# zxhuang1698/ZeroShape

Hardware: AMD Instinct MI355X
Metric: sdf_query_points_per_sec_vox128 (higher is better)
Workload: dtype f16x3

## Files before the change

include/zeroshape_hip.h:

```cpp
#ifndef ZEROSHAPE_HIP_H
#define ZEROSHAPE_HIP_H

#include <stddef.h>
#include <stdint.h>

#ifdef __cplusplus
extern "C" {
#endif

#define ZS_ABI_VERSION 40

int zs_abi_version(void);

const char *zs_last_error(void);


int zs_chamfer_forward(const float *xyz1, const float *xyz2, int b, int n, int m,
                       float *dist1, float *dist2, int *idx1, int *idx2, void *stream);

size_t zs_chamfer_workspace_bytes(int b, int n, int m);
int zs_chamfer_forward_ws(const float *xyz1, const float *xyz2, int b, int n, int m,
                          float *dist1, float *dist2, int *idx1, int *idx2,
                          void *workspace, size_t workspace_bytes, void *stream);

int zs_chamfer_backward(const float *xyz1, const float *xyz2, int b, int n, int m,
// ... 32 lines not shown
                           const float *axis, int G, const int *columns, int n_cols, float *zmean,
                           void *workspace, void *scratch, size_t scratch_bytes, void *stream);

int zs_attn_frames(const float *zmean, int batch, int n_cols, const int *frame_col, int n_frames,
                   const float *images, int H, int W, const uint8_t *lut, int R, float *frames, void *stream);

int zs_sdf_split_programs(const void *programs, size_t program_stride_bytes, void *split_programs,
                          size_t split_stride_bytes, int batch, void *stream);
int zs_sdf_query_points_split(const void *split_programs, size_t program_stride_bytes, int batch,
                              const float *points, int m, float *logits, int *tile_flags,
                              void *workspace, void *stream);
int zs_sdf_query_grid_split(const void *split_programs, size_t program_stride_bytes, int batch,
                            const float *axis, int G, int slice_begin, int slice_end,
                            int apply_sigmoid, float *out, int *tile_flags, void *workspace,
                            void *stream);

int zs_sdf_query_grid_range(const void *programs, size_t program_stride_bytes, int batch,
                            const float *axis, int G, long long point_begin, long long point_end,
                            int apply_sigmoid, float *out, const int *tile_mask, void *workspace,
                            void *stream);
int zs_sdf_query_grid_range_split(const void *split_programs, size_t program_stride_bytes, int batch,
                                  const float *axis, int G, long long point_begin,
                                  long long point_end, int apply_sigmoid, float *out,
                                  int *tile_flags, void *workspace, void *stream);

size_t zs_bf_grid_bytes(void);
size_t zs_bf_scratch_bytes(void);
int zs_bf_lower_bounds(const float *pred, int n, const float *gt_normalized, int m,
                       const float *rotations, int k, float *grid_gt, float *grid_pred,
                       void *scratch, float *lower_bounds, void *stream);
// ... 283 lines not shown
```

zeroshape_amd/_lib.py:

```python
import contextlib
import ctypes
import os

_HERE = os.path.dirname(os.path.abspath(__file__))
LIB_PATH = os.environ.get("ZS_LIB_PATH") or os.path.join(_HERE, "libzeroshape_hip.so")

_c_void_p = ctypes.c_void_p
_c_int = ctypes.c_int
_c_size_t = ctypes.c_size_t
_c_float = ctypes.c_float

class ConvFuse(ctypes.Structure):
    _fields_ = [("in_mode", ctypes.c_int), ("in_tiles", ctypes.c_int), ("in_groups", ctypes.c_int), ("in_gshift", ctypes.c_int),
                ("in_stats", ctypes.c_void_p), ("in_gamma", ctypes.c_void_p), ("in_beta", ctypes.c_void_p),
                ("in_eps", ctypes.c_float), ("out_mode", ctypes.c_int), ("out_groups", ctypes.c_int),
                ("out_stats", ctypes.c_void_p)]


SIGNATURES = {
    "zs_abi_version": (_c_int, []),
    "zs_last_error": (ctypes.c_char_p, []),
    "zs_chamfer_forward": (_c_int, [_c_void_p, _c_void_p, _c_int, _c_int, _c_int,
                                    _c_void_p, _c_void_p, _c_void_p, _c_void_p, _c_void_p]),
    "zs_chamfer_workspace_bytes": (_c_size_t, [_c_int, _c_int, _c_int]),
# ... 13 lines not shown
                                    _c_void_p, _c_int, _c_void_p]),
    "zs_sdf_verdict_stats": (_c_int, [_c_void_p, _c_void_p, _c_int, _c_int, _c_float, _c_float, _c_float, _c_void_p, _c_void_p,
                                      _c_void_p]),
    "zs_sdf_query_points": (_c_int, [_c_void_p, _c_size_t, _c_int, _c_void_p, _c_int,
                                     _c_void_p, _c_void_p, _c_void_p, _c_void_p, _c_void_p]),
    "zs_sdf_query_grid": (_c_int, [_c_void_p, _c_size_t, _c_int, _c_void_p, _c_int, _c_int,
                                   _c_int, _c_int, _c_void_p, _c_void_p, _c_void_p, _c_void_p]),
    "zs_sdf_grid_attn_zmean_scratch_bytes": (_c_size_t, [_c_int, _c_int, _c_int, _c_size_t]),
    "zs_sdf_grid_attn_zmean_chunk": (_c_int, [_c_int, _c_int, _c_int, _c_size_t, ctypes.POINTER(_c_int),
                                              ctypes.POINTER(_c_int)]),
    "zs_sdf_grid_attn_zmean": (_c_int, [_c_void_p, _c_size_t, _c_int, _c_void_p, _c_int, _c_void_p, _c_int, _c_void_p,
                                        _c_void_p, _c_void_p, _c_size_t, _c_void_p]),
    "zs_attn_frames": (_c_int, [_c_void_p, _c_int, _c_int, _c_void_p, _c_int, _c_void_p, _c_int, _c_int, _c_void_p, _c_int,
                                _c_void_p, _c_void_p]),
    "zs_sdf_split_programs": (_c_int, [_c_void_p, _c_size_t, _c_void_p, _c_size_t, _c_int, _c_void_p]),
    "zs_sdf_query_points_split": (_c_int, [_c_void_p, _c_size_t, _c_int, _c_void_p, _c_int,
                                           _c_void_p, _c_void_p, _c_void_p, _c_void_p]),
    "zs_sdf_query_grid_split": (_c_int, [_c_void_p, _c_size_t, _c_int, _c_void_p, _c_int, _c_int,
                                         _c_int, _c_int, _c_void_p, _c_void_p, _c_void_p, _c_void_p]),
    "zs_sdf_query_grid_range": (_c_int, [_c_void_p, _c_size_t, _c_int, _c_void_p, _c_int, ctypes.c_longlong,
                                         ctypes.c_longlong, _c_int, _c_void_p, _c_void_p, _c_void_p, _c_void_p]),
    "zs_sdf_query_grid_range_split": (_c_int, [_c_void_p, _c_size_t, _c_int, _c_void_p, _c_int,
                                               ctypes.c_longlong, ctypes.c_longlong, _c_int, _c_void_p,
                                               _c_void_p, _c_void_p, _c_void_p]),
    "zs_erode_mask": (_c_int, [_c_void_p, _c_int, _c_int, _c_int, _c_int, _c_void_p, _c_void_p]),
    "zs_bf_grid_bytes": (_c_size_t, []),
    "zs_bf_scratch_bytes": (_c_size_t, []),
    "zs_bf_lower_bounds": (_c_int, [_c_void_p, _c_int, _c_void_p, _c_int, _c_void_p, _c_int, _c_void_p,
                                    _c_void_p, _c_void_p, _c_void_p, _c_void_p]),
    "zs_pose_max_batch": (_c_int, []),
# ... 129 lines not shown
    "zs_group_norm_bwd_workspace_bytes": (_c_size_t, [_c_int, _c_int]),
    "zs_group_norm_bwd": (_c_int, [_c_void_p] * 8 + [_c_int, _c_int, _c_int, _c_int, _c_float, _c_void_p, _c_void_p]),
    "zs_max_pool_bwd_nhwc": (_c_int, [_c_void_p] * 3 + [_c_int] * 10 + [_c_void_p]),
    "zs_global_mean_bwd_nhwc": (_c_int, [_c_void_p, _c_void_p, _c_int, _c_int, _c_int, _c_void_p]),
    "zs_upsample2x_bwd_nhwc": (_c_int, [_c_void_p, _c_void_p, _c_int, _c_int, _c_int, _c_int, _c_void_p]),
    "zs_nhwc_to_nchw_masked": (_c_int, [_c_void_p, _c_void_p, _c_void_p, _c_int, _c_int, _c_int, _c_int, _c_void_p]),
    "zs_seen_surface_bwd": (_c_int, [_c_void_p] * 7 + [_c_int, _c_int, _c_int, _c_void_p, _c_void_p, _c_void_p]),
    "zs_intr_param2mtx_bwd": (_c_int, [_c_void_p, _c_void_p, _c_int, _c_int, _c_int, _c_void_p, _c_void_p]),
    "zs_window_tokens_bwd": (_c_int, [_c_void_p] * 5 + [_c_int] * 5 + [_c_void_p]),
    "zs_coord_dsp2_bwd": (_c_int, [_c_void_p] * 4 + [_c_int] * 3 + [_c_void_p]),
    "zs_transform_points": (_c_int, [_c_void_p] * 5 + [_c_int, _c_int, _c_void_p]),
    "zs_resize_bilinear_nhwc": (_c_int, [_c_void_p, _c_void_p] + [_c_int] * 6 + [_c_void_p]),
    "zs_readout_concat_bwd": (_c_int, [_c_void_p, _c_void_p, _c_int, _c_int, _c_int, _c_void_p]),
}

ABI_VERSION = 40
_lib = None


class ZeroShapeHipError(RuntimeError):
    pass


def load():
    global _lib
    if _lib is not None:
        return _lib
    if not os.path.exists(LIB_PATH):
        raise ZeroShapeHipError(
            "HIP library not built: %s is missing (run `python -m zeroshape_amd.build`). "
            "zeroshape_amd has no CPU/PyTorch fallback for this path." % LIB_PATH)
# ... 51 lines not shown
```

zeroshape_amd/csrc/sdf_decoder_split.hip:

```cpp
#include "zs_common.h"
#include <stdlib.h>
#include "sdf_layout.h"
#include "sdf_math.h"
#include "zs_split16.h"
#include "../../include/zeroshape_hip.h"

#include <math.h>
#include <stdint.h>
#include <type_traits>

namespace {

using namespace zs::lay;
using zs::dm::gelu_erf;
using zs::dm::softplus100;

typedef float f32x16 __attribute__((ext_vector_type(16)));
typedef float f32x4 __attribute__((ext_vector_type(4)));
typedef float f32x2 __attribute__((ext_vector_type(2)));
typedef unsigned u32x4 __attribute__((ext_vector_type(4)));

constexpr float S_GUARD = 64.0f;
constexpr int WAVES = 4;
constexpr int PTS_PER_WAVE = 32;
// ... 63 lines not shown
    asm volatile("s_mov_b32 m0, %1\n\ts_nop 0\n\tglobal_load_lds_dwordx4 %0, off" ZS_DMA_MOD
                 "\n\tglobal_load_lds_dwordx4 %0, off offset:1024" ZS_DMA_MOD
                 "\n\tglobal_load_lds_dwordx4 %0, off offset:2048" ZS_DMA_MOD
                 "\n\tglobal_load_lds_dwordx4 %0, off offset:3072" ZS_DMA_MOD
                 :
                 : "v"(gsrc), "s"(lds_dst)
                 : "memory");
}

struct AStream {
    const u32x4 *buf[NBUF];
    unsigned dst[NBUF];
    u32x4 hi, lo;
    const char *gsrc;

    DEV void init(const char *prog, u32x4 *stage, unsigned stage_addr, int wave, int lane) {
        const char *g = prog + wave * (KPW * KB_U4 * 16) + lane * 16;
        asm volatile("s_waitcnt vmcnt(0) lgkmcnt(0)\n\ts_barrier" ::: "memory");
#pragma unroll
        for (int i = 0; i < NBUF; i++) {
            buf[i] = stage + i * (CK * KB_U4) + lane;
            dst[i] = stage_addr + i * CHUNK_BYTES + wave * (KPW * KB_U4 * 16);
            glds_kblocks(g + i * CHUNK_BYTES, dst[i]);
        }
        gsrc = g + NBUF * CHUNK_BYTES;
        asm volatile("s_waitcnt vmcnt(4)\n\ts_barrier" ::: "memory");
        hi = buf[0][0];
        lo = buf[0][64];
    }
    template <int EXTRA_VM = 0>
    DEV void step(int pos, u32x4 &ahi, u32x4 &alo) {
        ahi = hi;
// ... 9 lines not shown
            const u32x4 *t = buf[0];
            const unsigned u = dst[0];
            buf[0] = buf[1];
            dst[0] = dst[1];
            buf[1] = t;
            dst[1] = u;
            hi = buf[0][0];
            lo = buf[0][64];
        } else {
#ifndef ZS_EXP_NO_AREAD
            hi = buf[0][(pos + 1) * KB_U4];
            lo = buf[0][(pos + 1) * KB_U4 + 64];
#endif
        }
    }
    DEV void drain() { asm volatile("s_waitcnt vmcnt(0) lgkmcnt(0)" ::: "memory"); }
};

struct Slab {
    u32x4 *fl;
    PT t7;
    DEV void store(int tile, const PT &p) {
        if (tile == SLAB_TILES) {
            t7 = p;
        } else {
#pragma unroll
            for (int q = 0; q < 4; q++) fl[(tile * 4 + q) * 64] = p.v[q];
        }
    }
};
// ... 124 lines not shown
#endif
                 "v_mul_f32_e64 %[t], |%[x]|, %[c0]\n\t"
                 "v_exp_f32_e32 %[t], %[t]\n\t"
                 "v_mfma_f32_32x32x16_f16 %[acc], %[ahi], %[bl], %[acc]\n\t"
                 "v_max_f32_e32 %[m], 0, %[x]\n\t"
                 "v_add_f32_e32 %[t], 1.0, %[t]\n\t"
                 "v_log_f32_e32 %[t], %[t]\n\t"
                 "v_mfma_f32_32x32x16_f16 %[acc], %[ahi], %[bh], %[acc]\n\t"
                 "s_nop 0\n\t"
                 "v_fmac_f32_e32 %[m], 0x3be32166, %[t]"
                 : [acc] "+v"(acc), [t] "=&v"(t), [m] "=&v"(m)
                 : [alo] "v"(alo), [ahi] "v"(ahi), [bh] "v"(bhi), [bl] "v"(blo), [x] "v"(x), [c0] "s"(c0));
    return m;
}

template <int KT, int EXTRA_VM = 0, typename SIDE = NoSide>
DEV void gemm_reg(AStream &s, const PT *X, f32x16 &acc, SIDE side = SIDE()) {
#pragma unroll
    for (int kt = 0; kt < KT; kt++)
#pragma unroll
        for (int j = 0; j < 2; j++) {
            u32x4 ahi, alo;
            s.step((kt * 2 + j) & (CK - 1), ahi, alo);
            pin(ahi, alo);
            mfma3_gaps(acc, ahi, alo, X[kt].v[2 * j], X[kt].v[2 * j + 1], kt * 2 + j, side);
        }
}
template <typename SIDE>
DEV void mfma3_breg(f32x16 &acc, const u32x4 &ahi, const u32x4 &alo, const u32x4 &bhi, const u32x4 &blo, int kb,
                    SIDE &side) {
// ... 139 lines not shown
    const f32x4 *q = reinterpret_cast<const f32x4 *>(prm + off + tile * 32 + hi * 16);
#pragma unroll
    for (int i = 0; i < 4; i++) {
        const f32x4 a = q[i];
        v[4 * i + 0] = a.x; v[4 * i + 1] = a.y; v[4 * i + 2] = a.z; v[4 * i + 3] = a.w;
    }
}
DEV f32x16 rp16(const float *prm, int off, int tile, int hi) {
    float t[16];
    rp(prm, off, tile, hi, t);
    f32x16 v;
#pragma unroll
    for (int r = 0; r < 16; r++) v[r] = t[r];
    return v;
}
DEV f32x16 xyz_affine(const float *prm, int off, int tile, int hi, float x, float y, float z) {
    const f32x4 *q = reinterpret_cast<const f32x4 *>(prm + off + tile * 128 + hi * 64);
    f32x16 v;
#pragma unroll
    for (int r = 0; r < 16; r++) {
        const f32x4 w = q[r];
        v[r] = fmaf(w.z, z, fmaf(w.y, y, fmaf(w.x, x, w.w)));
    }
    return v;
}

struct XyzInit {
    const f32x4 *q;
    f32x4 w;
    f32x16 v;
// ... 93 lines not shown
    for (int r = 0; r < 16; r++) {
        const float p = __builtin_amdgcn_exp2f(fmaf(S[r], c, -m_run));
        S[r] = p;
        zs_ += p;
    }
    z_run += zs_;
    gemm_one(s, pack_tile(S), o, pos0 + 2);
}

#ifdef ZS_EXP_TIMING
#define ZS_STAMP(i) do { if (dbg) dbg[i] = __builtin_amdgcn_s_memtime(); } while (0)
#else
#define ZS_STAMP(i) do { } while (0)
#endif
DEV float decode_tile(const char *prog, float *prm, u32x4 *stage, unsigned stage_addr, u32x4 *slab,
                      f32x4 *zs, float px, float py, float pz, int wave, int lane, float &guard,
                      unsigned long long *dbg) {
    const int hi = lane >> 5;
    const float *prog_params = reinterpret_cast<const float *>(prog) + REC_FLOATS;
    AStream s;
    s.init(prog, stage, stage_addr, wave, lane);
    Slab sl;
    sl.fl = slab;
    ZS_STAMP(0);

    load_params(prm, prog_params, W_PP, 1024);
    f32x16 y[NT];
#pragma unroll
    for (int kt = 0; kt < NT; kt++) y[kt] = xyz_affine(prm, 0, kt, hi, px, py, pz);

    ZS_STAMP(1);

    const float scale = 0.17677669529663688110f;

#pragma unroll 1
    for (int blk = 0; blk < BLOCKS; blk++) {
        load_params(prm, prog_params, W_BLK + blk * P_BLK_STRIDE, P_BLK_STRIDE);
        layer_norm_lds(y, sl, prm, PB_LN1G, PB_LN1B, hi);
        ZS_STAMP(2 + blk * 4);
#pragma unroll
        for (int nt = 0; nt < NT; nt++) y[nt] += rp16(prm, PB_BPROJ, nt, hi);

        auto head = [&](int hd, auto Ptag) {
            constexpr int P = decltype(Ptag)::value;
            f32x16 q = rp16(prm, PB_BQKV, hd * 3 + 0, hi);
            gemm_lds(s, sl, q, P);
            f32x16 k = rp16(prm, PB_BQKV, hd * 3 + 1, hi);
            gemm_lds(s, sl, k, P);
            f32x16 v = rp16(prm, PB_BQKV, hd * 3 + 2, hi);
            gemm_lds(s, sl, v, P);

            const float c = scale * 1.44269504088896340736f;
            float s_self = 0.f;
            float qq = 0.f;
#pragma unroll
            for (int r = 0; r < 16; r++) {
                s_self = fmaf(q[r], k[r], s_self);
                qq = fmaf(q[r], q[r], qq);
            }
            s_self = half_sum(s_self) * c;
            {
                const float km = prog_params[P_KMAX + blk * HEADS + hd] * scale;
                guard = fmaxf(guard, half_sum(qq) * (km * km));
            }
            const PT qp = pack_tile(q);
// ... 5 lines not shown
                attn_tile<false>(s, qp, o, m_run, z_run, c, hi, P);
                attn_tile<false>(s, qp, o, m_run, z_run, c, hi, (P + 4) & (CK - 1));
            }
            attn_tile<true>(s, qp, o, m_run, z_run, c, hi, P);
            {
                const float m_new = fmaxf(m_run, s_self);
                const float alpha = __builtin_amdgcn_exp2f(m_run - m_new);
                const float p_self = __builtin_amdgcn_exp2f(s_self - m_new);
                const float z = fmaf(half_sum(z_run), alpha, p_self);
                const float inv = 1.0f / z;
                const float a_i = alpha * inv, p_i = p_self * inv;
#pragma unroll
                for (int r = 0; r < 16; r++) o[r] = fmaf(p_i, v[r], o[r] * a_i);
            }
            const PT op = pack_tile(o);
#pragma unroll
            for (int nt = 0; nt < NT; nt++) gemm_one(s, op, y[nt], (P + 4 + 2 * nt) & (CK - 1));
        };
        static_assert((LT - 1) % 2 == 0 && (3 * NT * 2 + LT * 4 + NT * 2) % CK == 4, "head = 11.5 chunks");
#pragma unroll 1
        for (int hd = 0; hd < HEADS; hd += 2) {
            head(hd, std::integral_constant<int, 0>());
            head(hd + 1, std::integral_constant<int, 4>());
        }

        ZS_STAMP(3 + blk * 4);
        layer_norm_lds(y, sl, prm, PB_LN2G, PB_LN2B, hi);
#pragma unroll
        for (int nt = 0; nt < NT; nt++) y[nt] += rp16(prm, PB_B2, nt, hi);
        ZS_STAMP(4 + blk * 4);
        RowInit bi;
        f32x16 hid = rp16(prm, PB_B1, 0, hi);
        bi.start(prm, PB_B1, 1, hi);
        gemm_lds(s, sl, hid, 0, [&](int kb, int g) {
            if (g == 2 && (kb & 3) == 1) bi.step(kb & ~3);
        });
#pragma unroll 1
        for (int ht = 0; ht < HT - 1; ht++) {
            f32x16 nxt = bi.v;
            bi.start(prm, PB_B1, ht + 2 < HT ? ht + 2 : HT - 1, hi);
            TilePacker e;
// ... 38 lines not shown
        ini.v = xyz_affine(prm, P_IMPL0 - W_IA, 0, hi, px, py, pz);
#pragma unroll
        for (int nt = 0; nt <= NT; nt++) {
            TilePacker e;
            if (nt < NT) {
                f32x16 acc = ini.v;
                if (nt + 1 < NT) ini.start(prm, P_IMPL0 - W_IA, nt + 1, hi);
                if (nt > 0)
                    gemm_reg_act<1>(s, hp, acc, prev, [&](int kb, float r) { e.feed(kb, r); },
                                    [&](int kb) { if (nt + 1 < NT) ini.step(kb, px, py, pz); });
                else
                    gemm_reg<NT, 0>(s, hp, acc, [&](int kb, int g) { if (g == 2) ini.step(kb, px, py, pz); });
                if (nt > 0) sl.store(nt - 1, e.p);
                prev = acc;
            } else {
#pragma unroll
                for (int kb = 0; kb < 16; kb++) e.feed(kb, softplus100(prev[kb]));
                sl.store(nt - 1, e.p);
            }
        }
    }
    ZS_STAMP(11);
    const float rsqrt2 = 0.70710678118654752440f;
    PT fp[NT];
#pragma unroll
    for (int kt = 0; kt < NT; kt++) {
        float t[16];
#pragma unroll
        for (int r = 0; r < 16; r++) t[r] = h[kt * 16 + r] * rsqrt2;
        fp[kt] = pack_tile(t);
// ... 7 lines not shown
        ini.v = rp16(prm, P_IMPL1 - W_IA, 0, hi);
#pragma unroll
        for (int nt = 0; nt <= NT; nt++) {
            TilePacker e;
            if (nt < NT) {
                f32x16 acc = ini.v;
                if (nt + 1 < NT) ini.start(prm, P_IMPL1 - W_IA, nt + 1, hi);
                if (nt > 0)
                    gemm_lds_act<1>(s, sl, acc, prev, [&](int kb, float r) { e.feed(kb, r * rsqrt2); },
                                    [&](int kb) { if (nt + 1 < NT) ini.step(kb); });
                else
                    gemm_lds(s, sl, acc, 0, [&](int kb, int g) { if (g == 2) ini.step(kb); });
                if (nt > 0) hp[nt - 1] = e.p;
                prev = acc;
            } else {
#pragma unroll
                for (int kb = 0; kb < 16; kb++) e.feed(kb, softplus100(prev[kb]) * rsqrt2);
                hp[nt - 1] = e.p;
            }
        }
    }
    ZS_STAMP(13);
    float out = 0.f;
#pragma unroll 1
    for (int i = 0; i < 3; i++) {
        if (i == 1) load_params(prm, prog_params, W_IB, P_USED - W_IB);
        const int pp = i == 0 ? P_IMPL_PAIR - W_IA : (i - 1) * P_IMPL_PAIR_STRIDE;
        {
            f32x16 prev;
            XyzInit ini;
            ini.v = xyz_affine(prm, pp, 0, hi, sx, sy, sz);
#pragma unroll
            for (int nt = 0; nt <= NT; nt++) {
                TilePacker e;
                if (nt < NT) {
                    f32x16 acc = ini.v;
                    if (nt + 1 < NT) ini.start(prm, pp, nt + 1, hi);
                    if (nt > 0)
                        gemm_reg_act<1>(s, hp, acc, prev, [&](int kb, float r) { e.feed(kb, r); }, [&](int) {});
                    else
                        gemm_reg<NT>(s, hp, acc);
                    gemm_areg<NT>(s, fp, acc, [&](int kb, int g) {
                        if (g == 2 && nt + 1 < NT) ini.step(kb, sx, sy, sz);
                    });
                    if (nt > 0) sl.store(nt - 1, e.p);
                    prev = acc;
                } else {
#pragma unroll
                    for (int kb = 0; kb < 16; kb++) e.feed(kb, softplus100(prev[kb]));
// ... 21 lines not shown
                if (nt < NT) {
                    f32x16 acc = ini.v;
                    if (nt + 1 < NT) ini.start(prm, pp + 1024, nt + 1, hi);
                    w8.start(prm, P_W8 - W_IB, nt, hi);
                    auto tail = [&](int kb) {
                        if (nt + 1 < NT) ini.step(kb);
                        w8.step(kb);
                    };
                    if (nt > 0)
                        gemm_lds_act<1>(s, sl, acc, prev, [&](int kb, float r) { finish(kb, r); }, tail);
                    else
                        gemm_lds(s, sl, acc, 0, [&](int kb, int g) { if (g == 2) tail(kb); });
                    if (nt > 0) hp[nt - 1] = e.p;
                    prev = acc;
                } else {
#pragma unroll
                    for (int kb = 0; kb < 16; kb++) finish(kb, softplus100(prev[kb]));
                    hp[nt - 1] = e.p;
                }
            }
        }
    }
    ZS_STAMP(14);
    s.drain();
    out = half_sum(out);
    ZS_STAMP(15);
    return out + prm[P_B8 - W_IB];
}

template <bool GRID>
__global__ __launch_bounds__(WAVES * 64, 1) void sdf_decode_split_kernel(
    const char *__restrict__ programs, size_t program_stride_bytes, int batch,
    const float *__restrict__ points,
    const float *__restrict__ axis,
    int G, long long first_point,
    int m,
    float *__restrict__ out, int apply_sigmoid, f32x4 *__restrict__ workspace,
    int *__restrict__ tile_flags,
    int static_order) {
    __shared__ __attribute__((aligned(16))) float lds[LDS_FLOATS];
    float *prm = lds;
    const int lane = threadIdx.x & 63;
    const int wave = __builtin_amdgcn_readfirstlane(threadIdx.x >> 6);
    u32x4 *stage = reinterpret_cast<u32x4 *>(lds + PRM_WINDOW);
    const unsigned stage_addr = __builtin_amdgcn_readfirstlane(
        (unsigned)(uintptr_t)(__attribute__((address_space(3))) float *)(lds + PRM_WINDOW));
    u32x4 *fl = reinterpret_cast<u32x4 *>(lds + PRM_WINDOW + STAGE_FLOATS) + wave * SLAB_U4 + lane;
    f32x4 *zslab = workspace + ((size_t)blockIdx.x * WAVES + wave) * ZSLAB_F4 + lane;

    const int tiles_per_img = (m + PTS_PER_BLOCK - 1) / PTS_PER_BLOCK;
    const int total = tiles_per_img * batch;
    int *tile_counter = reinterpret_cast<int *>(workspace + (size_t)MAX_WGS * WAVES * ZSLAB_F4) + 256;
    int *tile_slot = tile_counter + 16 + blockIdx.x;
    const int dyn_tiles = total > (int)gridDim.x ? total - (int)gridDim.x : 0;
    for (int tile = blockIdx.x;;) {
      if (tile < total) {
        const int img = tile / tiles_per_img;
        const int t = tile - img * tiles_per_img;
        const char *prog = programs + (size_t)img * program_stride_bytes;

        const int p = t * PTS_PER_BLOCK + wave * PTS_PER_WAVE + (lane & 31);
        const int pc = p < m ? p : m - 1;
        float px, py, pz;
// ... 8 lines not shown
            py = axis[iy];
            pz = axis[iz];
        } else {
            const float *q = points + ((size_t)img * m + pc) * 3;
            px = q[0];
            py = q[1];
            pz = q[2];
        }
#ifdef ZS_EXP_TIMING
        unsigned long long *dbg = (blockIdx.x == 0 && threadIdx.x == 0 && tile == 0)
            ? reinterpret_cast<unsigned long long *>(workspace + (size_t)MAX_WGS * WAVES * ZSLAB_F4) : nullptr;
#else
        unsigned long long *dbg = nullptr;
#endif
        float guard = 0.f;
        float logit = decode_tile(prog, prm, stage, stage_addr, fl, zslab, px, py, pz, wave, lane, guard, dbg);
        if (apply_sigmoid) logit = 1.0f / (1.0f + expf(-logit));
        const unsigned bad = reinterpret_cast<const unsigned *>(prog)[REC_FLOATS + P_FLAG];
        const bool pt_bad = (__builtin_bit_cast(unsigned, px) & 0x7f800000u) == 0x7f800000u ||
                            (__builtin_bit_cast(unsigned, py) & 0x7f800000u) == 0x7f800000u ||
                            (__builtin_bit_cast(unsigned, pz) & 0x7f800000u) == 0x7f800000u;
        if (bad || pt_bad) logit = __builtin_bit_cast(float, 0x7fc00000u);
        if (tile_flags) {
            const bool over = !(__builtin_bit_cast(unsigned, guard) <= __builtin_bit_cast(unsigned, S_GUARD * S_GUARD));
            if (__builtin_amdgcn_ballot_w64(over || bad != 0) != 0 && lane == 0) tile_flags[tile] = 1;
        }
        if (lane < 32 && p < m) out[(size_t)img * m + p] = logit;
      }
        if (static_order) {
            tile += (int)gridDim.x;
            if (tile >= total) break;
// ... 93 lines not shown
            for (int g = 0; g < 4; g++) {
                const f32x4 v = reinterpret_cast<const f32x4 *>(kv + (lt * 8 + g) * GROUP_FLOATS)[(t & 31) + 32 * half];
                sq = fmaf(v.x, v.x, fmaf(v.y, v.y, fmaf(v.z, v.z, fmaf(v.w, v.w, sq))));
            }
    }
    red[t] = sq;
    __syncthreads();
    for (int o = 128; o > 0; o >>= 1) {
        if (t < o) red[t] = fmaxf(red[t], red[t + o]);
        __syncthreads();
    }
    if (t == 0)
        reinterpret_cast<float *>(dst + (size_t)img * dst_stride_u4)[REC_FLOATS + P_KMAX + bh] = sqrtf(red[0]);
}

int decode_grid_size(int batch, int m) {
    const long long tiles = (long long)batch * ((m + PTS_PER_BLOCK - 1) / PTS_PER_BLOCK);
    return (int)(tiles < MAX_WGS ? tiles : MAX_WGS);
}

bool check_programs(const char *what, const void *programs, size_t stride) {
    if (!programs) {
        zs::set_err("%s: null pointer", what);
        return false;
    }
    if (stride % 16 != 0 || stride < zs_sdf_program_bytes()) {
        zs::set_err("%s: bad program stride %zu", what, stride);
        return false;
    }
    return true;
// ... 16 lines not shown
    hipStream_t st = static_cast<hipStream_t>(stream);
    if (hipMemset2DAsync(static_cast<char *>(split_programs) + (size_t)(REC_FLOATS + P_FLAG) * 4, split_stride_bytes,
                         0, 16, batch, st) != hipSuccess) {
        zs::set_err("zs_sdf_split_programs: hipMemset2DAsync failed");
        return 0;
    }
    hipLaunchKernelGGL(split_program_kernel, dim3((elems + 255) / 256, batch), dim3(256), 0, st,
                       static_cast<const float *>(programs), program_stride_bytes / sizeof(float),
                       static_cast<u32x4 *>(split_programs), split_stride_bytes / sizeof(u32x4));
    hipLaunchKernelGGL(k_bound_kernel, dim3(BLOCKS * HEADS, batch), dim3(256), 0, st,
                       static_cast<const float *>(programs), program_stride_bytes / sizeof(float),
                       static_cast<u32x4 *>(split_programs), split_stride_bytes / sizeof(u32x4));
    return zs::check_launch("zs_sdf_split_programs") ? 1 : 0;
}

static int launch_counter_reset(void *workspace, hipStream_t st) {
    const char *e = getenv("ZS_SPLIT_STATIC_TILES");
    if (e && atoi(e) != 0) return 1;
    int *tile_counter = reinterpret_cast<int *>(static_cast<f32x4 *>(workspace) + (size_t)MAX_WGS * WAVES * ZSLAB_F4) + 256;
    (void)hipMemsetAsync(tile_counter, 0, sizeof(int), st);
    return 0;
}

extern "C" int zs_sdf_query_points_split(const void *split_programs, size_t program_stride_bytes,
                                         int batch, const float *points, int m, float *logits,
                                         int *tile_flags, void *workspace, void *stream) {
    if (batch < 0 || m < 0) {
        zs::set_err("zs_sdf_query_points_split: negative size (batch=%d m=%d)", batch, m);
        return 0;
    }
    if (batch == 0 || m == 0) return 1;
    if (!points || !logits || !workspace) {
        zs::set_err("zs_sdf_query_points_split: null pointer");
        return 0;
    }
    if (!check_programs("zs_sdf_query_points_split", split_programs, program_stride_bytes)) return 0;
    if ((long long)batch * ((m + PTS_PER_BLOCK - 1) / PTS_PER_BLOCK) > 0x7fffffffLL) {
        zs::set_err("zs_sdf_query_points_split: too many tiles");
        return 0;
    }
    const int static_order = launch_counter_reset(workspace, static_cast<hipStream_t>(stream));
    hipLaunchKernelGGL((sdf_decode_split_kernel<false>), dim3(decode_grid_size(batch, m)),
                       dim3(WAVES * 64), 0, static_cast<hipStream_t>(stream),
                       static_cast<const char *>(split_programs), program_stride_bytes, batch, points,
                       nullptr, 0, 0LL, m, logits, 0, static_cast<f32x4 *>(workspace), tile_flags, static_order);
    return zs::check_launch("zs_sdf_query_points_split") ? 1 : 0;
}

extern "C" int zs_sdf_query_grid_range_split(const void *split_programs, size_t program_stride_bytes,
                                             int batch, const float *axis, int G, long long point_begin,
                                             long long point_end, int apply_sigmoid, float *out,
                                             int *tile_flags, void *workspace, void *stream) {
    const long long P = (long long)G * G * G;
    if (batch < 0 || G <= 0 || point_begin < 0 || point_end > P || point_begin > point_end) {
        zs::set_err("zs_sdf_query_grid_range_split: bad range (batch=%d G=%d points=[%lld,%lld))", batch, G,
                    point_begin, point_end);
        return 0;
    }
    const long long mm = point_end - point_begin;
    if (batch == 0 || mm == 0) return 1;
    if (!axis || !out || !workspace) {
        zs::set_err("zs_sdf_query_grid_range_split: null pointer");
        return 0;
    }
    if (mm > 0x7fffffffLL - PTS_PER_BLOCK) {
        zs::set_err("zs_sdf_query_grid_range_split: %lld points per launch exceed 2^31; split the range", mm);
        return 0;
    }
    if (!check_programs("zs_sdf_query_grid_range_split", split_programs, program_stride_bytes)) return 0;
    const int m = (int)mm;
    const int static_order = launch_counter_reset(workspace, static_cast<hipStream_t>(stream));
    hipLaunchKernelGGL((sdf_decode_split_kernel<true>), dim3(decode_grid_size(batch, m)),
                       dim3(WAVES * 64), 0, static_cast<hipStream_t>(stream),
                       static_cast<const char *>(split_programs), program_stride_bytes, batch, nullptr,
                       axis, G, point_begin, m, out, apply_sigmoid, static_cast<f32x4 *>(workspace), tile_flags, static_order);
    return zs::check_launch("zs_sdf_query_grid_range_split") ? 1 : 0;
}

extern "C" int zs_sdf_query_grid_split(const void *split_programs, size_t program_stride_bytes,
                                       int batch, const float *axis, int G, int slice_begin,
                                       int slice_end, int apply_sigmoid, float *out, int *tile_flags,
                                       void *workspace, void *stream) {
    if (batch < 0 || G <= 0 || slice_begin < 0 || slice_end > G || slice_begin > slice_end) {
        zs::set_err("zs_sdf_query_grid_split: bad range (batch=%d G=%d slices=[%d,%d))", batch, G,
                    slice_begin, slice_end);
        return 0;
    }
    const long long mm = (long long)(slice_end - slice_begin) * G * G;
    if (batch == 0 || mm == 0) return 1;
    if (!axis || !out || !workspace) {
        zs::set_err("zs_sdf_query_grid_split: null pointer");
        return 0;
    }
    if (mm > 0x7fffffffLL - PTS_PER_BLOCK) {
        zs::set_err("zs_sdf_query_grid_split: %lld points per launch exceed 2^31; split the slab", mm);
        return 0;
    }
    if (!check_programs("zs_sdf_query_grid_split", split_programs, program_stride_bytes)) return 0;
    const int m = (int)mm;
    const int static_order = launch_counter_reset(workspace, static_cast<hipStream_t>(stream));
    hipLaunchKernelGGL((sdf_decode_split_kernel<true>), dim3(decode_grid_size(batch, m)),
                       dim3(WAVES * 64), 0, static_cast<hipStream_t>(stream),
                       static_cast<const char *>(split_programs), program_stride_bytes, batch, nullptr,
                       axis, G, (long long)slice_begin * G * G, m, out, apply_sigmoid,
                       static_cast<f32x4 *>(workspace), tile_flags, static_order);
    return zs::check_launch("zs_sdf_query_grid_split") ? 1 : 0;
}
```

zeroshape_amd/program.py:

```python
import numpy as np

C = 256
NT = C // 32
HEADS = 8
HD = 32
L = 197
LT = 7
HID = 1024
HT = HID // 32
BLOCKS = 2
MLP_LAYERS = 9
SKIP_IN = (2, 4, 6)
GROUP_FLOATS = 256
RING = 8

LANE = np.arange(64)
LANE_I = LANE & 31
LANE_HI = LANE >> 5


def row(r, hi):
    return (r & 3) + 8 * (r >> 2) + 4 * hi


# ... 331 lines not shown
    return wmax <= W_MAX, dict(max_abs_weight=wmax)


def latent_k_bounds(prog):
    prog = np.ascontiguousarray(prog, np.float32)
    out = np.zeros((BLOCKS, HEADS), np.float32)
    for blk in range(BLOCKS):
        for h in range(HEADS):
            o = kv_group_offset(blk, h) * GROUP_FLOATS
            g = prog[o:o + G_KV_HEAD * GROUP_FLOATS].reshape(LT, 8, 64, 4)[:, :4]
            rec = g.transpose(0, 1, 3, 2).reshape(LT, 16, 64)
            sq = (rec.astype(np.float64) ** 2).sum(1)
            row = sq[:, :32] + sq[:, 32:]
            out[blk, h] = np.sqrt(row.max())
    return out
```

Measured before the change: 75.92 million.

## Fold block-0 layernorm and QKV projection into per-image rank-4 tables

Block 0's input to the QKV projection is a layernorm of an affine function of the point xyz, so the QKV GEMM collapses to a 4-term affine map of (x·rstd, y·rstd, z·rstd, rstd). A new kernel precomputes these per-image tables in double precision. The decode kernel then skips streaming the block-0 QKV weight chunks and replaces three GEMMs per head with FMAs. It also adds s_nop padding (mfma_settle) before MFMA results are read in the MLP. This adds an extra launch per query and reuses the workspace for the tables, and it changes numerics slightly.

```diff
diff --git a/include/zeroshape_hip.h b/include/zeroshape_hip.h
--- a/include/zeroshape_hip.h
+++ b/include/zeroshape_hip.h
@@ -8,7 +8,7 @@
 extern "C" {
 #endif
 
-#define ZS_ABI_VERSION 40
+#define ZS_ABI_VERSION 41
 
 int zs_abi_version(void);
 
@@ -71,6 +71,8 @@
                             const float *axis, int G, int slice_begin, int slice_end,
                             int apply_sigmoid, float *out, int *tile_flags, void *workspace,
                             void *stream);
+
+int zs_sdf_block0_tables(const void *split_programs, size_t program_stride_bytes, int batch, float *tables, void *stream);
 
 int zs_sdf_query_grid_range(const void *programs, size_t program_stride_bytes, int batch,
                             const float *axis, int G, long long point_begin, long long point_end,
diff --git a/zeroshape_amd/_lib.py b/zeroshape_amd/_lib.py
--- a/zeroshape_amd/_lib.py
+++ b/zeroshape_amd/_lib.py
@@ -51,6 +51,7 @@
     "zs_attn_frames": (_c_int, [_c_void_p, _c_int, _c_int, _c_void_p, _c_int, _c_void_p, _c_int, _c_int, _c_void_p, _c_int,
                                 _c_void_p, _c_void_p]),
     "zs_sdf_split_programs": (_c_int, [_c_void_p, _c_size_t, _c_void_p, _c_size_t, _c_int, _c_void_p]),
+    "zs_sdf_block0_tables": (_c_int, [_c_void_p, _c_size_t, _c_int, _c_void_p, _c_void_p]),
     "zs_sdf_query_points_split": (_c_int, [_c_void_p, _c_size_t, _c_int, _c_void_p, _c_int,
                                            _c_void_p, _c_void_p, _c_void_p, _c_void_p]),
     "zs_sdf_query_grid_split": (_c_int, [_c_void_p, _c_size_t, _c_int, _c_void_p, _c_int, _c_int,
@@ -210,7 +211,7 @@
     "zs_readout_concat_bwd": (_c_int, [_c_void_p, _c_void_p, _c_int, _c_int, _c_int, _c_void_p]),
 }
 
-ABI_VERSION = 40
+ABI_VERSION = 41
 _lib = None
 
 
diff --git a/zeroshape_amd/csrc/sdf_decoder_split.hip b/zeroshape_amd/csrc/sdf_decoder_split.hip
--- a/zeroshape_amd/csrc/sdf_decoder_split.hip
+++ b/zeroshape_amd/csrc/sdf_decoder_split.hip
@@ -101,8 +101,8 @@
     u32x4 hi, lo;
     const char *gsrc;
 
-    DEV void init(const char *prog, u32x4 *stage, unsigned stage_addr, int wave, int lane) {
-        const char *g = prog + wave * (KPW * KB_U4 * 16) + lane * 16;
+    DEV void init(const char *prog, u32x4 *stage, unsigned stage_addr, int wave, int lane, int first_byte = 0) {
+        const char *g = prog + first_byte + wave * (KPW * KB_U4 * 16) + lane * 16;
         asm volatile("s_waitcnt vmcnt(0) lgkmcnt(0)\n\ts_barrier" ::: "memory");
 #pragma unroll
         for (int i = 0; i < NBUF; i++) {
@@ -142,6 +142,7 @@
 #endif
         }
     }
+    DEV void skip(int bytes) { gsrc += bytes; }
     DEV void drain() { asm volatile("s_waitcnt vmcnt(0) lgkmcnt(0)" ::: "memory"); }
 };
 
@@ -296,6 +297,8 @@
     return m;
 }
 
+DEV void mfma_settle(f32x16 &acc) { asm volatile("s_nop 7\n\ts_nop 3" : "+v"(acc)); }
+
 template <int KT, int EXTRA_VM = 0, typename SIDE = NoSide>
 DEV void gemm_reg(AStream &s, const PT *X, f32x16 &acc, SIDE side = SIDE()) {
 #pragma unroll
@@ -465,6 +468,18 @@
     for (int r = 0; r < 16; r++) v[r] = t[r];
     return v;
 }
+constexpr int B0_BPROJ = 0, B0_C = 256, B0_T = 1024;
+static_assert(B0_T + HEADS * 3 * 128 == PRM_WINDOW, "the block-0 table is exactly one params window");
+DEV f32x16 block0_qkv(const float *prm, int tile, int hi, float xr, float yr, float zr, float rstd) {
+    f32x16 v = rp16(prm, B0_C, tile, hi);
+    const f32x4 *q = reinterpret_cast<const f32x4 *>(prm + B0_T + tile * 128 + hi * 64);
+#pragma unroll
+    for (int r = 0; r < 16; r++) {
+        const f32x4 w = q[r];
+        v[r] = fmaf(w.z, zr, fmaf(w.y, yr, fmaf(w.x, xr, fmaf(w.w, rstd, v[r]))));
+    }
+    return v;
+}
 DEV f32x16 xyz_affine(const float *prm, int off, int tile, int hi, float x, float y, float z) {
     const f32x4 *q = reinterpret_cast<const f32x4 *>(prm + off + tile * 128 + hi * 64);
     f32x16 v;
@@ -588,12 +603,14 @@
 #define ZS_STAMP(i) do { } while (0)
 #endif
 DEV float decode_tile(const char *prog, float *prm, u32x4 *stage, unsigned stage_addr, u32x4 *slab,
-                      f32x4 *zs, float px, float py, float pz, int wave, int lane, float &guard,
+                      const float *tbl, float px, float py, float pz, int wave, int lane, float &guard,
                       unsigned long long *dbg) {
     const int hi = lane >> 5;
     const float *prog_params = reinterpret_cast<const float *>(prog) + REC_FLOATS;
+    constexpr int QKV_BYTES = 3 * NT * 2 / CK * CHUNK_BYTES;
+    static_assert(3 * NT * 2 % CK == 0, "AStream::skip passes whole chunks");
     AStream s;
-    s.init(prog, stage, stage_addr, wave, lane);
+    s.init(prog, stage, stage_addr, wave, lane, tbl ? QKV_BYTES : 0);
     Slab sl;
     sl.fl = slab;
     ZS_STAMP(0);
@@ -609,20 +626,38 @@
 
 #pragma unroll 1
     for (int blk = 0; blk < BLOCKS; blk++) {
-        load_params(prm, prog_params, W_BLK + blk * P_BLK_STRIDE, P_BLK_STRIDE);
-        layer_norm_lds(y, sl, prm, PB_LN1G, PB_LN1B, hi);
+        const bool tab = blk == 0 && tbl != nullptr;
+        float rstd0 = 0.f, xr = 0.f, yr = 0.f, zr = 0.f;
+        if (tab) {
+            load_params(prm, tbl, 0, PRM_WINDOW);
+            float mean;
+            ln_stats(y, mean, rstd0);
+            xr = px * rstd0;
+            yr = py * rstd0;
+            zr = pz * rstd0;
+        } else {
+            load_params(prm, prog_params, W_BLK + blk * P_BLK_STRIDE, P_BLK_STRIDE);
+            layer_norm_lds(y, sl, prm, PB_LN1G, PB_LN1B, hi);
+        }
         ZS_STAMP(2 + blk * 4);
 #pragma unroll
-        for (int nt = 0; nt < NT; nt++) y[nt] += rp16(prm, PB_BPROJ, nt, hi);
+        for (int nt = 0; nt < NT; nt++) y[nt] += rp16(prm, tab ? B0_BPROJ : PB_BPROJ, nt, hi);
 
         auto head = [&](int hd, auto Ptag) {
             constexpr int P = decltype(Ptag)::value;
-            f32x16 q = rp16(prm, PB_BQKV, hd * 3 + 0, hi);
-            gemm_lds(s, sl, q, P);
-            f32x16 k = rp16(prm, PB_BQKV, hd * 3 + 1, hi);
-            gemm_lds(s, sl, k, P);
-            f32x16 v = rp16(prm, PB_BQKV, hd * 3 + 2, hi);
-            gemm_lds(s, sl, v, P);
+            f32x16 q, k, v;
+            if (tab) {
+                q = block0_qkv(prm, hd * 3 + 0, hi, xr, yr, zr, rstd0);
+                k = block0_qkv(prm, hd * 3 + 1, hi, xr, yr, zr, rstd0);
+                v = block0_qkv(prm, hd * 3 + 2, hi, xr, yr, zr, rstd0);
+            } else {
+                q = rp16(prm, PB_BQKV, hd * 3 + 0, hi);
+                gemm_lds(s, sl, q, P);
+                k = rp16(prm, PB_BQKV, hd * 3 + 1, hi);
+                gemm_lds(s, sl, k, P);
+                v = rp16(prm, PB_BQKV, hd * 3 + 2, hi);
+                gemm_lds(s, sl, v, P);
+            }
 
             const float c = scale * 1.44269504088896340736f;
             float s_self = 0.f;
@@ -658,8 +693,13 @@
                 for (int r = 0; r < 16; r++) o[r] = fmaf(p_i, v[r], o[r] * a_i);
             }
             const PT op = pack_tile(o);
-#pragma unroll
-            for (int nt = 0; nt < NT; nt++) gemm_one(s, op, y[nt], (P + 4 + 2 * nt) & (CK - 1));
+            const bool bump = tab && hd + 1 < HEADS;
+            if (bump && (P == 4 || wave >= 2)) s.skip(QKV_BYTES);
+#pragma unroll
+            for (int nt = 0; nt < NT; nt++) {
+                if (P == 0 && nt == 2 && bump && wave < 2) s.skip(QKV_BYTES);
+                gemm_one(s, op, y[nt], (P + 4 + 2 * nt) & (CK - 1));
+            }
         };
         static_assert((LT - 1) % 2 == 0 && (3 * NT * 2 + LT * 4 + NT * 2) % CK == 4, "head = 11.5 chunks");
 #pragma unroll 1
@@ -669,6 +709,7 @@
         }
 
         ZS_STAMP(3 + blk * 4);
+        if (tab) load_params(prm, prog_params, W_BLK, P_BLK_STRIDE);
         layer_norm_lds(y, sl, prm, PB_LN2G, PB_LN2B, hi);
 #pragma unroll
         for (int nt = 0; nt < NT; nt++) y[nt] += rp16(prm, PB_B2, nt, hi);
@@ -737,6 +778,7 @@
                 if (nt > 0) sl.store(nt - 1, e.p);
                 prev = acc;
             } else {
+                mfma_settle(prev);
 #pragma unroll
                 for (int kb = 0; kb < 16; kb++) e.feed(kb, softplus100(prev[kb]));
                 sl.store(nt - 1, e.p);
@@ -774,6 +816,7 @@
                 if (nt > 0) hp[nt - 1] = e.p;
                 prev = acc;
             } else {
+                mfma_settle(prev);
 #pragma unroll
                 for (int kb = 0; kb < 16; kb++) e.feed(kb, softplus100(prev[kb]) * rsqrt2);
                 hp[nt - 1] = e.p;
@@ -793,6 +836,7 @@
 #pragma unroll
             for (int nt = 0; nt <= NT; nt++) {
                 TilePacker e;
+                if (nt > 0) mfma_settle(prev);
                 if (nt < NT) {
                     f32x16 acc = ini.v;
                     if (nt + 1 < NT) ini.start(prm, pp, nt + 1, hi);
@@ -844,6 +888,7 @@
                     if (nt > 0) hp[nt - 1] = e.p;
                     prev = acc;
                 } else {
+                    mfma_settle(prev);
 #pragma unroll
                     for (int kb = 0; kb < 16; kb++) finish(kb, softplus100(prev[kb]));
                     hp[nt - 1] = e.p;
@@ -867,7 +912,8 @@
     int m,
     float *__restrict__ out, int apply_sigmoid, f32x4 *__restrict__ workspace,
     int *__restrict__ tile_flags,
-    int static_order) {
+    int static_order,
+    const float *__restrict__ block0_tables) {
     __shared__ __attribute__((aligned(16))) float lds[LDS_FLOATS];
     float *prm = lds;
     const int lane = threadIdx.x & 63;
@@ -876,7 +922,6 @@
     const unsigned stage_addr = __builtin_amdgcn_readfirstlane(
         (unsigned)(uintptr_t)(__attribute__((address_space(3))) float *)(lds + PRM_WINDOW));
     u32x4 *fl = reinterpret_cast<u32x4 *>(lds + PRM_WINDOW + STAGE_FLOATS) + wave * SLAB_U4 + lane;
-    f32x4 *zslab = workspace + ((size_t)blockIdx.x * WAVES + wave) * ZSLAB_F4 + lane;
 
     const int tiles_per_img = (m + PTS_PER_BLOCK - 1) / PTS_PER_BLOCK;
     const int total = tiles_per_img * batch;
@@ -915,7 +960,8 @@
         unsigned long long *dbg = nullptr;
 #endif
         float guard = 0.f;
-        float logit = decode_tile(prog, prm, stage, stage_addr, fl, zslab, px, py, pz, wave, lane, guard, dbg);
+        const float *tbl = block0_tables ? block0_tables + (size_t)img * PRM_WINDOW : nullptr;
+        float logit = decode_tile(prog, prm, stage, stage_addr, fl, tbl, px, py, pz, wave, lane, guard, dbg);
         if (apply_sigmoid) logit = 1.0f / (1.0f + expf(-logit));
         const unsigned bad = reinterpret_cast<const unsigned *>(prog)[REC_FLOATS + P_FLAG];
         const bool pt_bad = (__builtin_bit_cast(unsigned, px) & 0x7f800000u) == 0x7f800000u ||
@@ -1039,6 +1085,77 @@
         reinterpret_cast<float *>(dst + (size_t)img * dst_stride_u4)[REC_FLOATS + P_KMAX + bh] = sqrtf(red[0]);
 }
 
+constexpr int B0_THREADS = 256;
+__global__ __launch_bounds__(B0_THREADS) void block0_window_kernel(const char *__restrict__ programs,
+                                                                   size_t program_stride_bytes, float *__restrict__ tables) {
+    __shared__ double red[B0_THREADS][5];
+    __shared__ double msum[64][4];
+    const int tile = blockIdx.x, img = blockIdx.y, t = threadIdx.x, wave = t >> 6, lane = t & 63, hl = lane >> 5;
+    const char *prog = programs + (size_t)img * program_stride_bytes;
+    const float *par = reinterpret_cast<const float *>(prog) + REC_FLOATS;
+    float *out = tables + (size_t)img * PRM_WINDOW;
+    if (t < 64) {
+#pragma unroll
+        for (int d = 0; d < 4; d++) {
+            double a = 0.0;
+#pragma unroll
+            for (int f = 0; f < 4; f++) a += (double)par[P_PP + (4 * t + f) * 4 + d];
+            msum[t][d] = a;
+        }
+    }
+    __syncthreads();
+    double m[4] = {0.0, 0.0, 0.0, 0.0};
+    for (int i = 0; i < 64; i++)
+#pragma unroll
+        for (int d = 0; d < 4; d++) m[d] += msum[i][d];
+#pragma unroll
+    for (int d = 0; d < 4; d++) m[d] *= 1.0 / C;
+    const int head = tile / 3, part = tile - head * 3;
+    const u32x4 *kb0 = reinterpret_cast<const u32x4 *>(prog) + (size_t)(head * (G_HEAD / 2) + part * 2 * NT) * KB_U4;
+    double acc[5] = {0.0, 0.0, 0.0, 0.0, 0.0};
+#pragma unroll
+    for (int k = 0; k < 4; k++) {
+        const int kb = 4 * wave + k;
+        const u32x4 h4 = kb0[kb * KB_U4 + lane], l4 = kb0[kb * KB_U4 + 64 + lane];
+        const int f0 = (kb >> 1) * 32 + hl * 16 + (kb & 1) * 8;
+#pragma unroll
+        for (int e = 0; e < 8; e++) {
+            const unsigned hw = h4[e >> 1] >> (16 * (e & 1)), lw = l4[e >> 1] >> (16 * (e & 1));
+            const double w = (double)(float)__builtin_bit_cast(_Float16, (unsigned short)hw) +
+                             (double)(float)__builtin_bit_cast(_Float16, (unsigned short)lw);
+            const double wg = w * (double)par[P_BLK0 + PB_LN1G + f0 + e];
+#pragma unroll
+            for (int d = 0; d < 4; d++) acc[d] += wg * ((double)par[P_PP + (f0 + e) * 4 + d] - m[d]);
+            acc[4] += w * (double)par[P_BLK0 + PB_LN1B + f0 + e];
+        }
+    }
+#pragma unroll
+    for (int d = 0; d < 5; d++) red[t][d] = acc[d];
+    __syncthreads();
+    if (t < 32) {
+        const int hh = (t >> 2) & 1, r = (t & 3) + 4 * (t >> 3), o = tile * 32 + hh * 16 + r;
+        double sum[5] = {0.0, 0.0, 0.0, 0.0, 0.0};
+        for (int w = 0; w < B0_THREADS / 64; w++)
+#pragma unroll
+            for (int d = 0; d < 5; d++) sum[d] += red[w * 64 + t][d] + red[w * 64 + 32 + t][d];
+#pragma unroll
+        for (int d = 0; d < 4; d++) out[B0_T + o * 4 + d] = (float)sum[d];
+        out[B0_C + o] = (float)(sum[4] + (double)par[P_BLK0 + PB_BQKV + o]);
+    }
+    if (tile < C / 32 && t < 32) out[B0_BPROJ + tile * 32 + t] = par[P_BLK0 + PB_BPROJ + tile * 32 + t];
+}
+
+const float *launch_block0_tables(const void *split_programs, size_t program_stride_bytes, int batch, void *workspace,
+                                  hipStream_t st) {
+    const char *e = getenv("ZS_SPLIT_BLOCK0_GEMM");
+    if (e && atoi(e) != 0) return nullptr;
+    if ((size_t)batch * PRM_WINDOW * sizeof(float) > (size_t)MAX_WGS * WAVES * ZSLAB_F4 * sizeof(f32x4)) return nullptr;
+    float *tables = static_cast<float *>(workspace);
+    hipLaunchKernelGGL(block0_window_kernel, dim3(HEADS * 3, batch), dim3(B0_THREADS), 0, st,
+                       static_cast<const char *>(split_programs), program_stride_bytes, tables);
+    return tables;
+}
+
 int decode_grid_size(int batch, int m) {
     const long long tiles = (long long)batch * ((m + PTS_PER_BLOCK - 1) / PTS_PER_BLOCK);
     return (int)(tiles < MAX_WGS ? tiles : MAX_WGS);
@@ -1085,6 +1202,23 @@
     return zs::check_launch("zs_sdf_split_programs") ? 1 : 0;
 }
 
+extern "C" int zs_sdf_block0_tables(const void *split_programs, size_t program_stride_bytes, int batch, float *tables,
+                                    void *stream) {
+    if (batch < 0 || batch > 65535) {
+        zs::set_err("zs_sdf_block0_tables: bad batch %d", batch);
+        return 0;
+    }
+    if (batch == 0) return 1;
+    if (!tables) {
+        zs::set_err("zs_sdf_block0_tables: null pointer");
+        return 0;
+    }
+    if (!check_programs("zs_sdf_block0_tables", split_programs, program_stride_bytes)) return 0;
+    hipLaunchKernelGGL(block0_window_kernel, dim3(HEADS * 3, batch), dim3(B0_THREADS), 0, static_cast<hipStream_t>(stream),
+                       static_cast<const char *>(split_programs), program_stride_bytes, tables);
+    return zs::check_launch("zs_sdf_block0_tables") ? 1 : 0;
+}
+
 static int launch_counter_reset(void *workspace, hipStream_t st) {
     const char *e = getenv("ZS_SPLIT_STATIC_TILES");
     if (e && atoi(e) != 0) return 1;
@@ -1111,10 +1245,11 @@
         return 0;
     }
     const int static_order = launch_counter_reset(workspace, static_cast<hipStream_t>(stream));
+    const float *b0_tables = launch_block0_tables(split_programs, program_stride_bytes, batch, workspace, static_cast<hipStream_t>(stream));
     hipLaunchKernelGGL((sdf_decode_split_kernel<false>), dim3(decode_grid_size(batch, m)),
                        dim3(WAVES * 64), 0, static_cast<hipStream_t>(stream),
                        static_cast<const char *>(split_programs), program_stride_bytes, batch, points,
-                       nullptr, 0, 0LL, m, logits, 0, static_cast<f32x4 *>(workspace), tile_flags, static_order);
+                       nullptr, 0, 0LL, m, logits, 0, static_cast<f32x4 *>(workspace), tile_flags, static_order, b0_tables);
     return zs::check_launch("zs_sdf_query_points_split") ? 1 : 0;
 }
 
@@ -1141,10 +1276,11 @@
     if (!check_programs("zs_sdf_query_grid_range_split", split_programs, program_stride_bytes)) return 0;
     const int m = (int)mm;
     const int static_order = launch_counter_reset(workspace, static_cast<hipStream_t>(stream));
+    const float *b0_tables = launch_block0_tables(split_programs, program_stride_bytes, batch, workspace, static_cast<hipStream_t>(stream));
     hipLaunchKernelGGL((sdf_decode_split_kernel<true>), dim3(decode_grid_size(batch, m)),
                        dim3(WAVES * 64), 0, static_cast<hipStream_t>(stream),
                        static_cast<const char *>(split_programs), program_stride_bytes, batch, nullptr,
-                       axis, G, point_begin, m, out, apply_sigmoid, static_cast<f32x4 *>(workspace), tile_flags, static_order);
+                       axis, G, point_begin, m, out, apply_sigmoid, static_cast<f32x4 *>(workspace), tile_flags, static_order, b0_tables);
     return zs::check_launch("zs_sdf_query_grid_range_split") ? 1 : 0;
 }
 
@@ -1170,10 +1306,11 @@
     if (!check_programs("zs_sdf_query_grid_split", split_programs, program_stride_bytes)) return 0;
     const int m = (int)mm;
     const int static_order = launch_counter_reset(workspace, static_cast<hipStream_t>(stream));
+    const float *b0_tables = launch_block0_tables(split_programs, program_stride_bytes, batch, workspace, static_cast<hipStream_t>(stream));
     hipLaunchKernelGGL((sdf_decode_split_kernel<true>), dim3(decode_grid_size(batch, m)),
                        dim3(WAVES * 64), 0, static_cast<hipStream_t>(stream),
                        static_cast<const char *>(split_programs), program_stride_bytes, batch, nullptr,
                        axis, G, (long long)slice_begin * G * G, m, out, apply_sigmoid,
-                       static_cast<f32x4 *>(workspace), tile_flags, static_order);
+                       static_cast<f32x4 *>(workspace), tile_flags, static_order, b0_tables);
     return zs::check_launch("zs_sdf_query_grid_split") ? 1 : 0;
 }
diff --git a/zeroshape_amd/program.py b/zeroshape_amd/program.py
--- a/zeroshape_amd/program.py
+++ b/zeroshape_amd/program.py
@@ -369,3 +369,71 @@
             row = sq[:, :32] + sq[:, 32:]
             out[blk, h] = np.sqrt(row.max())
     return out
+
+
+B0_WINDOW_FLOATS = 4096
+B0_BPROJ, B0_C, B0_T = 0, C, C + HEADS * 96
+KB_HEAD = G_HEAD // 2
+KB_QKV_HEAD = G_QKV_HEAD // 2
+
+
+def _kblock_values(words, kb):
+    h = np.ascontiguousarray(words[kb * KB_WORDS:(kb + 1) * KB_WORDS]).view(np.float16).reshape(2, 64, 8)
+    return h[0].astype(np.float64) + h[1].astype(np.float64)
+
+
+def block0_qkv_weights(split_prog):
+    W = np.zeros((3 * C, C), np.float64)
+    for h in range(HEADS):
+        for part in range(3):
+            for kt in range(NT):
+                for j in range(2):
+                    v = _kblock_values(split_prog, h * KB_HEAD + part * 2 * NT + kt * 2 + j)
+                    rows = part * C + h * HD + LANE_I
+                    cols = 32 * kt + ROW_TABLE[LANE_HI][:, 8 * j:8 * j + 8]
+                    W[rows[:, None], cols] = v
+    return W
+
+
+def _from_rowparam(v):
+    v = np.asarray(v)
+    T = v.shape[0] // 32
+    idx = ((32 * np.arange(T))[:, None, None] + ROW_TABLE[None, :, :]).reshape(-1)
+    out = np.empty_like(v)
+    out[idx] = v
+    return out
+
+
+def block0_window(split_prog):
+    words = np.ascontiguousarray(split_prog).view(np.uint32)
+    params = words[REC_FLOATS:].view(np.float32).astype(np.float64)
+    d = PARAMS.blk[0]
+    A = np.stack([_from_rowparam(params[PARAMS.PP + i:PARAMS.PP + 4 * C:4]) for i in range(4)], axis=1)
+    g = _from_rowparam(params[d["ln1_g"]:d["ln1_g"] + C])
+    b = _from_rowparam(params[d["ln1_b"]:d["ln1_b"] + C])
+    W = block0_qkv_weights(words)
+    T = W @ (g[:, None] * (A - A.mean(axis=0, keepdims=True)))
+    c = W @ b
+    out = np.zeros(B0_WINDOW_FLOATS, np.float64)
+    out[B0_BPROJ:B0_BPROJ + C] = params[d["bproj"]:d["bproj"] + C]
+    for h in range(HEADS):
+        for part in range(3):
+            tile = 3 * h + part
+            rows = slice(part * C + h * HD, part * C + (h + 1) * HD)
+            out[B0_C + tile * 32:B0_C + (tile + 1) * 32] = \
+                _rowparam64(c[rows]) + params[d["bqkv"] + tile * 32:d["bqkv"] + (tile + 1) * 32]
+            out[B0_T + tile * 128:B0_T + (tile + 1) * 128] = \
+                np.stack([_rowparam64(T[rows, i]) for i in range(4)], axis=-1).reshape(-1)
+    return out.astype(np.float32)
+
+
+def _rowparam64(v):
+    v = np.asarray(v, np.float64)
+    T = v.shape[0] // 32
+    idx = (32 * np.arange(T))[:, None, None] + ROW_TABLE[None, :, :]
+    return v[idx].reshape(-1)
+
+
+def split_consumed_kblocks():
+    keep = [kb for kb in range(KB_TOTAL) if not (kb < HEADS * KB_HEAD and kb % KB_HEAD < KB_QKV_HEAD)]
+    return np.array(keep)
```

New measurement: 80.84 million (median of 6 runs). 1.06x the previous value.
